# VitalyVorobyev/calibration

Measured on AMD Instinct MI355X. Metric: residual+Jacobian evals/sec, higher is better.
Workload: dtype f64

## Files before the change

calibration_amd/csrc/backend_hip.hip:

```cpp
#include <rccl/rccl.h>

#include <atomic>
#include <cstring>
#include <mutex>
#include <thread>
#include <set>

#include "engine.hpp"
#include "pipelines.hpp"
#include "lm_core.hpp"
#include "lm_state.hpp"
#include "lm_kernels.hpp"

namespace cba {


static inline unsigned nblk(int64_t n, int per) { return static_cast<unsigned>(std::max<int64_t>(1, (n + per - 1) / per)); }

template <class F>
struct ScopeExit {
    F f;
    ~ScopeExit() { f(); }
};
template <class F>
// ... 739 lines not shown
    st->pin_pack[1].reserve(e.pk_size);
    {
        hipFuncAttributes fa;
        (void)hipFuncGetAttributes(&fa, reinterpret_cast<const void*>(k_schur_view));
        warm_reproj_kernels();
    }
    if (const char* env = std::getenv("CBA_SYRK_MFMA")) st->syrk_mfma = std::atoi(env);
    if (const char* env = cba_exp_env("CBA_SCHUR_WAVE")) st->schur_wave = std::atoi(env);
    if (const char* env = cba_exp_env("CBA_LM_FUSE")) st->fuse_small = std::atoi(env);
    if (const char* env = cba_exp_env("CBA_LM_CTL_EVENT")) st->ctl_event = std::atoi(env);
    if (const char* env = cba_exp_env("CBA_SYNC_SPIN")) st->sync_spin = std::atoi(env);
    if (const char* env = std::getenv("CBA_LM_GRAPH")) {
        const int v = std::atoi(env);
        st->graphs_ok = v != 0;
        st->graph_after = v > 1 ? v : (v == 1 ? 0 : st->graph_after);
    }
    e.blk_w.alloc(std::max(1, s.n_blocks));
    e.cam_acc.alloc(static_cast<size_t>(s.n_cams) * s.NACC);
    e.view_L.alloc(nv * 36);
    e.view_y.alloc(nv * 6);
    e.view_D.alloc(nv * 6);
    e.view_gp.alloc(nv * 6);
    e.view_scale2.alloc(nv * 6);
    e.view_fixed.alloc(nv);
    e.view_fixed.zero(e.stream);
    e.blk_Z.alloc(static_cast<size_t>(std::max(1, s.n_blocks)) * 6 * s.PSH);
    e.blk_Z.zero(e.stream);
    up64(st->cam_off, s.cam_off);
    st->res_active.alloc(std::max(1, s.nsh));
    st->res_cam_var.alloc(std::max(1, s.n_cams));
    st->res_Hcc.alloc(static_cast<size_t>(s.nsh) * s.nsh);
    st->res_Ssch.alloc(static_cast<size_t>(s.nsh) * s.nsh);
    st->res_out.alloc(32);
    if (const char* env = cba_exp_env("CBA_LM_CTL")) st->lm_ctl_mode = std::atoi(env) != 0;
    if (const char* env = cba_exp_env("CBA_LM_CTL_POLL_US")) st->ctl_poll_us = std::atoi(env);
    if (const char* env = cba_exp_env("CBA_LM_PRELAUNCH")) st->ctl_prelaunch = std::atoi(env);
    if (const char* env = std::getenv("CBA_RCCL_TIMEOUT_S")) st->rccl_timeout_s = std::max(1, std::atoi(env));
    warm_lm_ctl();
    if (const char* env = std::getenv("CBA_LM_RESIDENT")) st->resident_mode = std::atoi(env);
    if (const char* env = std::getenv("CBA_LM_RESIDENT_MAX_OBS")) st->resident_max_obs = std::atoll(env);
    CBA_HIP(hipStreamSynchronize(e.stream));
}

void solve_stats(const Engine& e, int64_t stats8[8]) {
    const HipLMState* st = reinterpret_cast<const HipLMState*>(e.lm_state);
    for (int k = 0; k < 8; ++k) stats8[k] = st ? st->xs[k] : 0;
}

void set_lm_mode(Engine& e, int mode) {
    if (mode < 0 || mode > 3)
        throw std::invalid_argument("lm mode: 0 chip-wide kernels, 1 automatic, 2 resident kernel whenever possible, 3 chip-wide kernels with the host-side iteration (diagnosis)");
    lm_state(e)->resident_mode = mode == 3 ? 0 : mode;
    lm_state(e)->lm_ctl_mode = mode == 3 ? 0 : 1;
}


static LMDriver make_driver(Engine& e, HipBackend& be) {
    AllReduce ar = [&e](double* buf, int64_t n) { engine_allreduce(e, buf, n); };
    return LMDriver(lm_state(e)->s, be, e.h_intr, e.h_cam, e.h_view, e.h_target, ar, e.n_ranks, e.rank);
}

void warm_lm(Engine& e) {
    cba_options o{};
    o.max_iterations = 1;
    const bool resident = resident_lm_eligible(e, o);
    {
// ... 99 lines not shown
```

calibration_amd/csrc/lm_state.hpp:

```cpp
#pragma once
#include "engine.hpp"
#include "lm_ctl.hpp"
#include "schur_math.hpp"
#include "structure.hpp"

namespace cba {

struct HipLMState {
    Structure s;
    SchurDims dims;
    int n_vchunks = 0, n_tiles = 0, n_pairs = 0, n_cchunks = 0;
    int fuse_small = 1;
    int schur_wave = 1;
    int syrk_mfma = 1;
    DevBuf<int32_t> view_cam_blk, cam_blk;
    DevBuf<int64_t> cchunk_off, cam_seg, link_off;
    DevBuf<int32_t> link_blk;
    DevBuf<double> cam_partial, view_gmax, view_delta, view_stats, syrk_partial;
    PinnedBuf<double> pin, pin_ne, pin_tr;
    DevBuf<double> pack_dev, sys_tiles, stat_dev;
    PinnedBuf<double> pin_packed;
    hipEvent_t step_done = nullptr;
    hipEvent_t ctl_done = nullptr;
    int ctl_event = 0;
    int sync_spin = 1;
    ~HipLMState() {
        if (step_done) (void)hipEventDestroy(step_done);
        if (ctl_done) (void)hipEventDestroy(ctl_done);
    }
    int64_t xs[8] = {0, 0, 0, 0, 0, 0, 0, 0};
    struct GraphSlot {
        hipGraphExec_t exec = nullptr;
        double huber = 0.0;
        int constrained = -1, scalar = -1;
        int uses = 0;
        ~GraphSlot() { if (exec) (void)hipGraphExecDestroy(exec); }
    };
    GraphSlot g_new, g_schur, g_trial;
    bool graphs_ok = true;
    int graph_after = 200;
    PinnedBuf<double> pin_lmp;
    PinnedBuf<double> pin_pack[2];
    bool current_is_on_device = false;
    int resident_mode = 1;
    int64_t resident_max_obs = -1;
    DevBuf<int64_t> cam_off;
    DevBuf<int8_t> res_active, res_cam_var;
    DevBuf<double> res_Hcc, res_Ssch, res_out;
    PinnedBuf<double> pin_res;
    PinnedBuf<int8_t> pin_mask;
    DevBuf<double> ctl_buf;
    DevBuf<int32_t> ctl_idx;
    DevBuf<int8_t> ctl_eff;
    PinnedBuf<double> ctl_rec;
    CtlView ctl_view{};
    int ctl_n = -1;
    int rccl_timeout_s = 120;
    int ctl_prelaunch = 1;
    int ctl_poll_us = 2000;
    int lm_ctl_mode = 1;
};


inline HipLMState* lm_state(Engine& e) { return reinterpret_cast<HipLMState*>(e.lm_state); }

bool resident_lm_eligible(const Engine& e, const cba_options& o);
void resident_lm_warm(Engine& e);
bool resident_lm_solve(Engine& e, const cba_options& o, cba_summary* out, bool keep_parameters = false);

void launch_lm_ctl(const CtlView& V, int mode, int flag, hipStream_t stream);
bool lm_ctl_fits_lds(int n);
void warm_lm_ctl();

}
```

calibration_amd/csrc/resident_lm.hip:

```cpp
#include <chrono>
#include <cstdio>
#include <cstdlib>
#include <cstring>

#include "engine.hpp"
#include "lm_core.hpp"
#include "lm_state.hpp"
#include "mode_b.hpp"
#include "schur_math.hpp"

namespace cba {

constexpr int RES_THREADS = 512, RES_WAVES = RES_THREADS / 64;
constexpr int RES_NSH_MAX = 80;
constexpr int RES_MAX_CAMS = 16;
constexpr int RES_PROF = 16;

struct ResidentArgs {
    int n_blocks, n_cams, n_views, nsh, n_tiles, sh_base;
    SchurDims dims;
    const Tile* tiles;
    const int64_t *blk_tile_off, *link_off, *cam_off;
    const int32_t *blk_cam, *blk_view, *link_blk, *view_cam_blk, *cam_blk, *view_fixed;
    const double *X, *Y, *u, *v, *aux;
    double *bc, *sd;
    double *intr[2], *cam[2], *view[2], *target[2];
    double *partial, *blk_acc, *blk_s, *blk_w, *cam_acc;
    double *view_L, *view_y, *view_D, *view_gp, *view_scale2, *blk_Z, *view_delta;
    double *Hcc, *Ssch;
    const int8_t *active, *cam_var;
    int intr_var, target_var, constrained, line_search;
    double huber, eps;
    int max_iterations;
    double* out;
};

enum ResidentMsg { MSG_GRADIENT = 0, MSG_MAX_ITER, MSG_MIN_RADIUS, MSG_INVALID_STEPS, MSG_PARAMETER, MSG_FUNCTION, MSG_LINE_SEARCH };
static const char* const kResidentMsg[] = {"Gradient tolerance reached.", "Maximum number of iterations reached.",
                                           "Minimum trust region radius reached.",
                                           "Number of consecutive invalid steps more than max.", "Parameter tolerance reached.",
                                           "Function tolerance reached."};

struct ResidentShared {
    double A[RES_NSH_MAX][RES_NSH_MAX + 1];
    double rhs[RES_NSH_MAX], delta[RES_NSH_MAX], gc[RES_NSH_MAX], gsch[RES_NSH_MAX], scale2[RES_NSH_MAX];
    int idx[RES_NSH_MAX];
    int8_t eff[RES_NSH_MAX];
    double red[RES_WAVES][6];
    double grp[RES_THREADS];
    double radius, decrease_factor, cost, gmax, gmax_priv;
    int m, nfail, valid;
    unsigned long long prof[RES_PROF];
    double p_intr[2][RES_MAX_CAMS * 12], p_cam[2][RES_MAX_CAMS * 7], p_target[2][7];
};

template <int N>
__device__ __forceinline__ void block_sum(double (&v)[N], ResidentShared& sh) {
    const int lane = threadIdx.x & 63, wave = threadIdx.x >> 6;
#pragma unroll
    for (int k = 0; k < N; ++k) {
        const double t = wave_sum63(v[k]);
        if (lane == 63) sh.red[wave][k] = t;
    }
    __syncthreads();
#pragma unroll
    for (int k = 0; k < N; ++k) {
        double t = 0.0;
        for (int w = 0; w < RES_WAVES; ++w) t += sh.red[w][k];
        v[k] = t;
    }
    __syncthreads();
}

__device__ __forceinline__ double block_max(double v, ResidentShared& sh) {
    for (int o = 32; o > 0; o >>= 1) v = fmax(v, __shfl_xor(v, o));
    if ((threadIdx.x & 63) == 0) sh.red[threadIdx.x >> 6][0] = v;
    __syncthreads();
    double m = sh.red[0][0];
    for (int w = 1; w < RES_WAVES; ++w) m = fmax(m, sh.red[w][0]);
    __syncthreads();
    return m;
}

template <class NT, class TF, class OF>
// ... 122 lines not shown
        if (CHAIN == CH_INTRINSIC) {
            pA = a.view[which] + 7 * static_cast<int64_t>(a.blk_view[b]);
        } else if (CHAIN == CH_EXTRINSIC) {
            pA = a.view[which] + 7 * static_cast<int64_t>(a.blk_view[b]);
            pB = sh.p_cam[which] + 7 * a.blk_cam[b];
        } else {
            pA = sh.p_target[which];
            pB = sh.p_cam[which] + 7 * a.blk_cam[b];
            ax = a.aux + 12 * static_cast<int64_t>(b);
        }
        double o[BC_SIZE];
        block_consts<CHAIN>(pA, pB, ax, o);
        for (int i = 0; i < BC_SIZE; ++i) a.bc[static_cast<int64_t>(b) * BC_SIZE + i] = o[i];
    }
    if (MODEL == CAM_SCHEIMPFLUG)
        for (int c = threadIdx.x; c < a.n_cams; c += RES_THREADS) {
            double o[SD_SIZE];
            for (int i = 0; i < SD_SIZE; ++i) o[i] = 0.0;
            scheimpflug_consts(sh.p_intr[which] + 12 * c, o);
            for (int i = 0; i < SD_SIZE; ++i) a.sd[static_cast<int64_t>(c) * SD_SIZE + i] = o[i];
        }
    __syncthreads();
}

template <int CHAIN, int MODEL, int NPARTS, int PART>
struct ModeBParts {
    static __device__ __forceinline__ void run(const Tile t, int lane, const double* bcp, const double* ip, const double* sp,
                                               const ResidentArgs& a, double* row) {
        normal_eq_tile<CHAIN, MODEL, NPARTS, PART, double>(t, lane, bcp, ip, sp, a.X, a.Y, a.u, a.v, row);
        if constexpr (PART + 1 < NPARTS) ModeBParts<CHAIN, MODEL, NPARTS, PART + 1>::run(t, lane, bcp, ip, sp, a, row);
    }
};

template <int CHAIN, int MODEL>
__device__ __forceinline__ void phase_mode_b(const ResidentArgs& a) {
    constexpr int PI = IntrSize<MODEL>::value;
    constexpr int NACC = LocalCols<CHAIN, MODEL>::value * (LocalCols<CHAIN, MODEL>::value + 1) / 2 + LocalCols<CHAIN, MODEL>::value + 1;
    constexpr int NPARTS = CHAIN == CH_INTRINSIC ? 3 : 6;
    const int lane = threadIdx.x & 63;
    const int wave = __builtin_amdgcn_readfirstlane(threadIdx.x >> 6);
    const bool direct = a.n_tiles == a.n_blocks;
    for (int w = wave; w < a.n_tiles; w += RES_WAVES) {
        const Tile t = a.tiles[w];
        const int cam = a.blk_cam[t.blk];
        double* row = (direct ? a.blk_acc : a.partial) + static_cast<int64_t>(w) * NACC;
        ModeBParts<CHAIN, MODEL, NPARTS, 0>::run(t, lane, a.bc + static_cast<int64_t>(t.blk) * BC_SIZE, a.intr[0] + static_cast<int64_t>(cam) * PI,
                                                 a.sd + static_cast<int64_t>(cam) * SD_SIZE, a, row);
    }
    __syncthreads();
    if (!direct) {
        for (int idx = threadIdx.x; idx < a.n_blocks * NACC; idx += RES_THREADS) {
            const int b = idx / NACC, e = idx - b * NACC;
            double s = 0.0;
            for (int64_t t = a.blk_tile_off[b]; t < a.blk_tile_off[b + 1]; ++t) s += a.partial[t * NACC + e];
            a.blk_acc[idx] = s;
        }
        __syncthreads();
    }
}

template <int MODEL>
__device__ __forceinline__ double phase_resid_cost(const ResidentArgs& a, int which, ResidentShared& sh) {
    constexpr int PI = IntrSize<MODEL>::value;
    const int lane = threadIdx.x & 63;
    const int wave = __builtin_amdgcn_readfirstlane(threadIdx.x >> 6);
    for (int w = wave; w < a.n_tiles; w += RES_WAVES) {
        const Tile t = a.tiles[w];
        const int cam = a.blk_cam[t.blk];
        const double s = resid_tile<MODEL, double>(t, lane, a.bc + static_cast<int64_t>(t.blk) * BC_SIZE,
                                                   a.intr[which] + static_cast<int64_t>(cam) * PI, a.sd + static_cast<int64_t>(cam) * SD_SIZE,
                                                   a.X, a.Y, a.u, a.v);
        if (lane == 63) a.partial[w] = s;
    }
    __syncthreads();
    double c[1] = {0.0};
    for (int b = threadIdx.x; b < a.n_blocks; b += RES_THREADS) {
        double s = 0.0;
        for (int64_t t = a.blk_tile_off[b]; t < a.blk_tile_off[b + 1]; ++t) s += a.partial[t];
        a.blk_s[b] = s;
        double rho, w;
        huber(s, a.huber, &rho, &w);
        c[0] += 0.5 * rho;
    }
    block_sum(c, sh);
    return c[0];
}

__device__ __forceinline__ double phase_weights(const ResidentArgs& a, ResidentShared& sh) {
    const int NACC = a.dims.NACC, s_idx = a.dims.NH + a.dims.PL;
    double c[1] = {0.0};
    for (int b = threadIdx.x; b < a.n_blocks; b += RES_THREADS) {
        double rho, w;
        huber(a.blk_acc[static_cast<int64_t>(b) * NACC + s_idx], a.huber, &rho, &w);
        a.blk_w[b] = w;
        c[0] += 0.5 * rho;
    }
    block_sum(c, sh);
    grouped_sums(
        a.n_cams * NACC, [&](int idx) { const int cam = idx / NACC; return static_cast<int>(a.cam_off[cam + 1] - a.cam_off[cam]); },
        [&](int idx, int k) {
            const int cam = idx / NACC, e = idx - cam * NACC;
            const int b = a.cam_blk[a.cam_off[cam] + k];
            return a.blk_w[b] * a.blk_acc[static_cast<int64_t>(b) * NACC + e];
        },
        [&](int idx, double s) { a.cam_acc[idx] = s; }, sh);
    return c[0];
}

__device__ __forceinline__ void phase_assemble(const ResidentArgs& a, bool init_scale, ResidentShared& sh) {
    const int n = a.nsh, PL = a.dims.PL, NACC = a.dims.NACC, NH = a.dims.NH;
    for (int idx = threadIdx.x; idx < n * n + n; idx += RES_THREADS) {
        if (idx < n * n) {
            const int i = idx / n, j = idx - i * n;
            int ci, li, cj, lj;
            shared_decode(a, i, &ci, &li);
            shared_decode(a, j, &cj, &lj);
            double h = 0.0;
            if (ci < 0 && cj < 0) {
                for (int c = 0; c < a.n_cams; ++c) h += a.cam_acc[static_cast<int64_t>(c) * NACC + hidx_sym(PL, li, lj)];
            } else if (ci < 0 || cj < 0 || ci == cj) {
                h = a.cam_acc[static_cast<int64_t>(ci < 0 ? cj : ci) * NACC + hidx_sym(PL, li, lj)];
            }
            a.Hcc[idx] = h;
        } else {
            const int i = idx - n * n;
            int ci, li;
            shared_decode(a, i, &ci, &li);
            double g = 0.0;
            if (ci < 0) {
                for (int c = 0; c < a.n_cams; ++c) g += a.cam_acc[static_cast<int64_t>(c) * NACC + NH + li];
            } else {
                g = a.cam_acc[static_cast<int64_t>(ci) * NACC + NH + li];
            }
            sh.gc[i] = g;
        }
    }
    __syncthreads();
    for (int i = threadIdx.x; i < n; i += RES_THREADS) {
        const double hii = a.Hcc[static_cast<int64_t>(i) * n + i];
        sh.eff[i] = a.active[i] && hii != 0.0;
        if (init_scale) {
            const double sc = 1.0 / (1.0 + sqrt(hii));
            sh.scale2[i] = sc * sc;
        }
    }
    __syncthreads();
    if (threadIdx.x == 0) {
        int m = 0;
        for (int i = 0; i < n; ++i)
            if (sh.eff[i]) sh.idx[m++] = i;
        sh.m = m;
    }
}

template <class Tick>
__device__ __forceinline__ void phase_schur(const ResidentArgs& a, bool init_scale, ResidentShared& sh, Tick tick) {
    const int n = a.nsh;
    double gm = 0.0, nf[1] = {0.0};
    const double radius = sh.radius;
    for (int v = threadIdx.x; v < a.n_views; v += RES_THREADS) {
        const int nb = static_cast<int>(a.link_off[v + 1] - a.link_off[v]);
        double g = 0.0;
        const bool ok = schur_view_body(a.dims, nb, a.link_blk + a.link_off[v], a.blk_acc, a.blk_w, a.view_fixed[v] != 0, radius, init_scale,
                                        a.constrained != 0, a.view[0] + 7 * static_cast<int64_t>(v), a.view_scale2 + 6 * static_cast<int64_t>(v),
                                        a.view_L + 36 * static_cast<int64_t>(v), a.view_y + 6 * static_cast<int64_t>(v),
                                        a.view_D + 6 * static_cast<int64_t>(v), a.view_gp + 6 * static_cast<int64_t>(v), a.blk_Z, &g);
        if (ok) gm = fmax(gm, g);
        else nf[0] += 1.0;
    }
    tick(11);
    gm = block_max(gm, sh);
    block_sum(nf, sh);
    tick(12);
    if (threadIdx.x == 0) { sh.gmax_priv = gm; sh.nfail = static_cast<int>(nf[0] + 0.5); }
    const int PC = a.dims.PC, PSH = a.dims.PSH, n_cams = a.n_cams;
    grouped_sums(
        n * n, [&](int) { return a.n_views; },
        [&](int idx, int v) {
            const int i = idx / n, j = idx - i * n;
            const int ci = i / PC, cj = j / PC;
            const int bi = a.view_cam_blk[static_cast<int64_t>(v) * n_cams + ci], bj = a.view_cam_blk[static_cast<int64_t>(v) * n_cams + cj];
            if (bi < 0 || bj < 0) return 0.0;
            const double* zi = a.blk_Z + static_cast<int64_t>(bi) * 6 * PSH + (i - ci * PC);
            const double* zj = a.blk_Z + static_cast<int64_t>(bj) * 6 * PSH + (j - cj * PC);
            double s = 0.0;
#pragma unroll
            for (int k = 0; k < 6; ++k) s += zi[k * PSH] * zj[k * PSH];
            return s;
        },
        [&](int idx, double s) { a.Ssch[idx] = s; }, sh);
    tick(13);
    grouped_sums(
        n, [&](int) { return a.n_views; },
        [&](int i, int v) {
            const int ci = i / PC;
            const int bi = a.view_cam_blk[static_cast<int64_t>(v) * n_cams + ci];
// ... 84 lines not shown
}

template <int CHAIN, int MODEL>
__global__ __launch_bounds__(RES_THREADS) void k_resident_lm(const ResidentArgs a) {
    __shared__ ResidentShared sh;
    const int tid = threadIdx.x;
    const int n = a.nsh;
    const double eps = a.eps;
    constexpr double min_radius = 1e-32, max_radius = 1e16, min_rel_decrease = 1e-3;

    unsigned long long last = wall_clock64();
    auto tick = [&](int slot) {
        if (tid == 0) {
            const unsigned long long t = wall_clock64();
            sh.prof[slot] += t - last;
            last = t;
        }
    };
    {
        const int PI = IntrSize<MODEL>::value;
        for (int i = tid; i < a.n_cams * PI; i += RES_THREADS) {
            double x = a.intr[0][i];
            if (a.intr_var && i % PI < 2) x = fmax(x, 0.0);
            sh.p_intr[0][i] = x;
        }
        if (CHAIN != CH_INTRINSIC)
            for (int i = tid; i < a.n_cams * 7; i += RES_THREADS) sh.p_cam[0][i] = a.cam[0][i];
        if (CHAIN == CH_BUNDLE)
            for (int i = tid; i < 7; i += RES_THREADS) sh.p_target[0][i] = a.target[0][i];
        if (tid == 0) {
            for (int k = 0; k < RES_PROF; ++k) sh.prof[k] = 0;
            sh.radius = 1e4;
            sh.decrease_factor = 2.0;
        }
        __syncthreads();
        publish_shared(a, sh, 0, 0);
    }
    double initial_cost = 0.0;
    int iter = 0, invalid = 0, successful = 0, term = CBA_TERM_FAILURE, msg = MSG_INVALID_STEPS;
    bool linearise = true, re_eliminate = false, first = true;
    while (true) {
        if (linearise) {
            phase_consts<CHAIN, MODEL>(a, sh, 0);
            tick(0);
            phase_mode_b<CHAIN, MODEL>(a);
            tick(1);
            const double cost = phase_weights(a, sh);
            tick(2);
            phase_assemble(a, first, sh);
            tick(3);
            if (tid == 0) sh.cost = cost;
        }
        if (linearise || re_eliminate) {
            phase_schur(a, first && linearise, sh, tick);
            tick(4);
        }
        if (linearise) {
            const double gm_shared = shared_gmax(a, sh);
            if (tid == 0) sh.gmax = fmax(sh.gmax_priv, gm_shared);
            __syncthreads();
            tick(5);
        }
        linearise = re_eliminate = false;
        if (first) {
            first = false;
            initial_cost = sh.cost;
            if (sh.gmax <= eps) { term = CBA_TERM_CONVERGENCE; msg = MSG_GRADIENT; break; }
        }
        if (iter >= a.max_iterations) { term = CBA_TERM_NO_CONVERGENCE; msg = MSG_MAX_ITER; break; }
        if (sh.gmax <= eps) { term = CBA_TERM_CONVERGENCE; msg = MSG_GRADIENT; break; }
        if (sh.radius <= min_radius) { term = CBA_TERM_CONVERGENCE; msg = MSG_MIN_RADIUS; break; }
        ++iter;
        tick(10);
        phase_solve_reduced(a, sh);
        tick(6);
        bool valid = sh.valid != 0;
        if (valid) {
            double st[6] = {0.0, 0.0, 0.0, 0.0, 0.0, 0.0};
            shared_plus(a, sh, sh.delta, &st[0], &st[1]);
            for (int v = tid; v < a.n_views; v += RES_THREADS) {
                const int nb = static_cast<int>(a.link_off[v + 1] - a.link_off[v]);
                double o4[4];
                backsub_view_body(a.dims, nb, a.link_blk + a.link_off[v], a.blk_cam, a.blk_Z, sh.delta, a.view_fixed[v] != 0,
                                  a.view_L + 36 * static_cast<int64_t>(v), a.view_y + 6 * static_cast<int64_t>(v),
                                  a.view_D + 6 * static_cast<int64_t>(v), a.view_gp + 6 * static_cast<int64_t>(v),
                                  a.view[0] + 7 * static_cast<int64_t>(v), a.view_delta + 6 * static_cast<int64_t>(v),
                                  a.view[1] + 7 * static_cast<int64_t>(v), o4);
                for (int k = 0; k < 4; ++k) st[k] += o4[k];
            }
            for (int i = RES_THREADS - 1 - tid; i < n; i += RES_THREADS) {
                const double di = sh.delta[i];
                if (di != 0.0) {
                    st[4] += sh.gc[i] * di;
                    double s = 0.0;
                    for (int j = 0; j < n; ++j) s += a.Hcc[static_cast<int64_t>(i) * n + j] * sh.delta[j];
                    st[5] += di * s;
                }
            }
            block_sum(st, sh);
            tick(7);
            const double model_change = -(st[2] + st[4]) - 0.5 * (st[3] + st[5]);
            if (!(model_change > 0.0) || !(fabs(model_change) <= 1.7976931348623157e308)) valid = false;
            if (valid) {
                publish_shared(a, sh, 1, 1, false);
                phase_consts<CHAIN, MODEL>(a, sh, 1);
                double cand = phase_resid_cost<MODEL>(a, 1, sh);
                tick(8);
                if (!(fabs(cand) <= 1.7976931348623157e308)) cand = 1.7976931348623157e308;
                if (a.constrained && a.line_search && !(cand <= sh.cost + 1e-4 * (st[2] + st[4]))) { term = CBA_TERM_FAILURE; msg = MSG_LINE_SEARCH; break; }
                const double step_norm = sqrt(st[0]), x_norm = sqrt(st[1]);
                if (step_norm <= eps * (x_norm + eps)) { term = CBA_TERM_CONVERGENCE; msg = MSG_PARAMETER; break; }
                const double cost_change = sh.cost - cand;
                if (fabs(cost_change) <= eps * sh.cost) { term = CBA_TERM_CONVERGENCE; msg = MSG_FUNCTION; break; }
                const double rel = cost_change / model_change;
                invalid = 0;
                if (rel > min_rel_decrease) {
                    publish_shared(a, sh, 1, 0);
                    for (int i = tid; i < a.n_views * 7; i += RES_THREADS) a.view[0][i] = a.view[1][i];
                    ++successful;
                    __syncthreads();
                    if (tid == 0) {
                        const double t = 2.0 * rel - 1.0;
                        sh.radius = fmin(max_radius, sh.radius / fmax(1.0 / 3.0, 1.0 - t * t * t));
                        sh.decrease_factor = 2.0;
                    }
                    __syncthreads();
                    tick(9);
                    linearise = true;
                } else {
                    __syncthreads();
                    if (tid == 0) {
                        sh.radius = sh.radius / sh.decrease_factor;
                        sh.decrease_factor *= 2.0;
                    }
                    __syncthreads();
                    re_eliminate = true;
                }
                continue;
            }
        }
        if (++invalid >= 5) { term = CBA_TERM_FAILURE; msg = MSG_INVALID_STEPS; break; }
        __syncthreads();
        if (tid == 0) sh.radius *= 0.5;
        __syncthreads();
        re_eliminate = true;
    }
    __syncthreads();
    phase_consts<CHAIN, MODEL>(a, sh, 0);
    if (tid == 0) {
        a.out[0] = term;
        a.out[1] = iter;
        a.out[2] = successful;
        a.out[3] = initial_cost;
        a.out[4] = sh.cost;
        a.out[5] = msg;
        tick(10);
        for (int k = 0; k < RES_PROF; ++k) a.out[8 + k] = static_cast<double>(sh.prof[k]);
    }
}

bool resident_lm_eligible(const Engine& e, const cba_options& o) {
    const HipLMState* st = reinterpret_cast<const HipLMState*>(e.lm_state);
    if (!st || st->resident_mode == 0) return false;
    const Structure& s = st->s;
    if (e.n_ranks != 1 || e.allreduce || e.rccl_comm) return false;
    if (e.scalar != 0 || o.verbose) return false;
    if (s.n_blocks == 0 || s.nsh > RES_NSH_MAX || s.n_cams > RES_MAX_CAMS) return false;
    if (st->resident_mode == 1) {
        if (st->resident_max_obs >= 0) return s.n_obs <= st->resident_max_obs;
        if (s.chain == CBA_CHAIN_INTRINSIC) return 1.0 * s.n_views + 0.0105 * static_cast<double>(s.n_obs) <= 28.0;
        return false;
    }
    return true;
}

static ResidentArgs resident_args(Engine& e, HipLMState& st) {
    const Structure& s = st.s;
    ResidentArgs a{};
    a.n_blocks = s.n_blocks; a.n_cams = s.n_cams; a.n_views = s.n_views; a.nsh = s.nsh;
    a.n_tiles = static_cast<int>(e.n_tilesB); a.sh_base = s.sh_base;
    a.dims = st.dims;
    a.tiles = e.tilesB.p; a.blk_tile_off = e.d_blk_tile_off.p; a.link_off = st.link_off.p; a.cam_off = st.cam_off.p;
    a.blk_cam = e.d_blk_cam.p; a.blk_view = e.d_blk_view.p; a.link_blk = st.link_blk.p; a.view_cam_blk = st.view_cam_blk.p;
    a.cam_blk = st.cam_blk.p; a.view_fixed = e.view_fixed.p;
    a.X = e.X.p; a.Y = e.Y.p; a.u = e.u.p; a.v = e.v.p; a.aux = e.aux.p;
    a.bc = e.bc.p; a.sd = e.sd.p;
    for (int k = 0; k < 2; ++k) { a.intr[k] = e.intr[k].p; a.cam[k] = e.cam[k].p; a.view[k] = e.view[k].p; a.target[k] = e.target[k].p; }
    a.partial = e.partial.p; a.blk_acc = e.blk_acc.p; a.blk_s = e.blk_s.p; a.blk_w = e.blk_w.p; a.cam_acc = e.cam_acc.p;
    a.view_L = e.view_L.p; a.view_y = e.view_y.p; a.view_D = e.view_D.p; a.view_gp = e.view_gp.p; a.view_scale2 = e.view_scale2.p;
    a.blk_Z = e.blk_Z.p; a.view_delta = st.view_delta.p;
    a.Hcc = st.res_Hcc.p; a.Ssch = st.res_Ssch.p;
    a.active = st.res_active.p; a.cam_var = st.res_cam_var.p;
    a.out = st.res_out.p;
    return a;
}

static void resident_launch(Engine& e, const ResidentArgs& a) {
#define CALL(C, M) hipLaunchKernelGGL((k_resident_lm<C, M>), dim3(1), dim3(RES_THREADS), 0, e.stream, a);
    switch (e.chain * 2 + e.model) {
        case 0: CALL(CH_INTRINSIC, CAM_PINHOLE_BC) break;
        case 1: CALL(CH_INTRINSIC, CAM_SCHEIMPFLUG) break;
        case 2: CALL(CH_EXTRINSIC, CAM_PINHOLE_BC) break;
        case 3: CALL(CH_EXTRINSIC, CAM_SCHEIMPFLUG) break;
        case 4: CALL(CH_BUNDLE, CAM_PINHOLE_BC) break;
        case 5: CALL(CH_BUNDLE, CAM_SCHEIMPFLUG) break;
        default: throw std::runtime_error("bad chain/model");
    }
#undef CALL
    CBA_HIP(hipGetLastError());
}

void resident_lm_warm(Engine& e) {
    HipLMState& st = *lm_state(e);
    cba_options o{};
    o.max_iterations = 0;
    o.huber_delta = 1.0;
    o.epsilon = 1e-9;
    if (!resident_lm_eligible(e, o)) return;
    cba_summary s{};
    resident_lm_solve(e, o, &s, true);
    (void)st;
// ... 33 lines not shown
    a.huber = o.huber_delta; a.eps = o.epsilon; a.max_iterations = o.max_iterations;
    a.line_search = 1;
    if (const char* env = std::getenv("CBA_LM_LINE_SEARCH")) a.line_search = std::atoi(env) != 0;
    resident_launch(e, a);
    const size_t n_intr = e.h_intr.size(), n_cam = e.h_cam.size(), n_view = e.h_view.size();
    st.pin_res.reserve(8 + n_intr + n_cam + 7 + n_view + RES_PROF);
    double* p = st.pin_res.p;
    st.res_out.download(p, 8, e.stream);
    double* prof = p + 8 + n_intr + n_cam + 7 + n_view;
    st.res_out.download(prof, RES_PROF, e.stream, 8);
    e.intr[0].download(p + 8, n_intr, e.stream);
    if (e.chain != CBA_CHAIN_INTRINSIC) e.cam[0].download(p + 8 + n_intr, n_cam, e.stream);
    if (e.chain == CBA_CHAIN_BUNDLE) e.target[0].download(p + 8 + n_intr + n_cam, 7, e.stream);
    if (n_view) e.view[0].download(p + 8 + n_intr + n_cam + 7, n_view, e.stream);
    CBA_HIP(hipStreamSynchronize(e.stream));
    e.active = 0;
    if (static_cast<int>(p[5]) == MSG_LINE_SEARCH) {
        if (!e.h_view.empty()) e.view[0].upload(e.h_view.data(), e.h_view.size(), e.stream);
        e.intr[0].upload(e.h_intr.data(), e.h_intr.size(), e.stream);
        if (e.chain != CBA_CHAIN_INTRINSIC) e.cam[0].upload(e.h_cam.data(), e.h_cam.size(), e.stream);
        if (e.chain == CBA_CHAIN_BUNDLE) e.target[0].upload(e.h_target.data(), 7, e.stream);
        CBA_HIP(hipStreamSynchronize(e.stream));
        return false;
    }
    if (!keep_parameters) {
        std::memcpy(e.h_intr.data(), p + 8, sizeof(double) * n_intr);
        if (e.chain != CBA_CHAIN_INTRINSIC) std::memcpy(e.h_cam.data(), p + 8 + n_intr, sizeof(double) * n_cam);
        if (e.chain == CBA_CHAIN_BUNDLE) std::memcpy(e.h_target.data(), p + 8 + n_intr + n_cam, sizeof(double) * 7);
        if (n_view) std::memcpy(e.h_view.data(), p + 8 + n_intr + n_cam + 7, sizeof(double) * n_view);
    }
    if (std::getenv("CBA_LM_RESIDENT_PROFILE")) {
        static const char* const names[RES_PROF] = {"consts", "mode B", "weights + camera sums", "assemble", "schur", "gradient norm",
                                                    "reduced solve", "trial step", "trial cost", "accept", "control", "schur: views",
                                                    "schur: max", "schur: S", "", ""};
        std::fprintf(stderr, "[cba] resident LM phases (us):");
        for (int k = 0; k < RES_PROF - 2; ++k) std::fprintf(stderr, " %s %.1f |", names[k], prof[k] * 0.01);
        std::fprintf(stderr, "\n");
    }
    const int term = static_cast<int>(p[0]), msg = static_cast<int>(p[5]);
    out->termination = term;
    out->success = term == CBA_TERM_CONVERGENCE;
    out->iterations = static_cast<int>(p[1]);
    out->successful_steps = static_cast<int>(p[2]);
    out->initial_cost = p[3];
    out->final_cost = p[4];
    out->solve_seconds = std::chrono::duration<double>(std::chrono::steady_clock::now() - t0).count();
    std::snprintf(out->report, sizeof(out->report), "calibba(schur LM, resident kernel): %s iters=%d cost %.6e -> %.6e",
                  kResidentMsg[msg >= 0 && msg < 6 ? msg : 3], out->iterations, out->initial_cost, out->final_cost);
    return true;
}

}
```

Baseline: 27.72 billion.

## Speculatively linearise at trial point in resident LM with double-buffered block accumulators

Each trial step in the resident LM kernel now runs the full mode-B Jacobian accumulation at the trial parameters instead of only computing the residual cost. The block accumulators and weights are double-buffered, so an accepted step flips a selector and reuses the trial linearisation instead of recomputing it. For the intrinsic chain, mode-B work is split into fixed 128-point units processed by wave pairs that exchange Jacobian rows through LDS, with next-unit loads prefetched. The trade is extra work on rejected steps (speculation is turned off after a rejection) plus additional device buffers and a larger shared-memory union.

New measurement: 27.71 billion, median of 4. About the same (-0.0%).

```diff
diff --git a/calibration_amd/csrc/backend_hip.hip b/calibration_amd/csrc/backend_hip.hip
--- a/calibration_amd/csrc/backend_hip.hip
+++ b/calibration_amd/csrc/backend_hip.hip
@@ -795,6 +795,7 @@
     st->res_Hcc.alloc(static_cast<size_t>(s.nsh) * s.nsh);
     st->res_Ssch.alloc(static_cast<size_t>(s.nsh) * s.nsh);
     st->res_out.alloc(32);
+    resident_lm_init(e);
     if (const char* env = cba_exp_env("CBA_LM_CTL")) st->lm_ctl_mode = std::atoi(env) != 0;
     if (const char* env = cba_exp_env("CBA_LM_CTL_POLL_US")) st->ctl_poll_us = std::atoi(env);
     if (const char* env = cba_exp_env("CBA_LM_PRELAUNCH")) st->ctl_prelaunch = std::atoi(env);
diff --git a/calibration_amd/csrc/lm_state.hpp b/calibration_amd/csrc/lm_state.hpp
--- a/calibration_amd/csrc/lm_state.hpp
+++ b/calibration_amd/csrc/lm_state.hpp
@@ -47,6 +47,10 @@
     DevBuf<int64_t> cam_off;
     DevBuf<int8_t> res_active, res_cam_var;
     DevBuf<double> res_Hcc, res_Ssch, res_out;
+    DevBuf<Tile> res_units;
+    DevBuf<int32_t> res_blk_unit_off;
+    DevBuf<double> res_rows;
+    int res_n_units = 0;
     PinnedBuf<double> pin_res;
     PinnedBuf<int8_t> pin_mask;
     DevBuf<double> ctl_buf;
@@ -64,6 +68,7 @@
 
 inline HipLMState* lm_state(Engine& e) { return reinterpret_cast<HipLMState*>(e.lm_state); }
 
+void resident_lm_init(Engine& e);
 bool resident_lm_eligible(const Engine& e, const cba_options& o);
 void resident_lm_warm(Engine& e);
 bool resident_lm_solve(Engine& e, const cba_options& o, cba_summary* out, bool keep_parameters = false);
diff --git a/calibration_amd/csrc/resident_lm.hip b/calibration_amd/csrc/resident_lm.hip
--- a/calibration_amd/csrc/resident_lm.hip
+++ b/calibration_amd/csrc/resident_lm.hip
@@ -14,6 +14,9 @@
 constexpr int RES_THREADS = 512, RES_WAVES = RES_THREADS / 64;
 constexpr int RES_NSH_MAX = 80;
 constexpr int RES_MAX_CAMS = 16;
+constexpr int RES_PAIRS = RES_WAVES / 2;
+constexpr int RES_UNIT = 128;
+constexpr int RES_ROW_NR2 = 16;
 constexpr int RES_PROF = 16;
 
 struct ResidentArgs {
@@ -25,7 +28,11 @@
     const double *X, *Y, *u, *v, *aux;
     double *bc, *sd;
     double *intr[2], *cam[2], *view[2], *target[2];
-    double *partial, *blk_acc, *blk_s, *blk_w, *cam_acc;
+    double *blk_acc[2], *blk_w[2], *sub[2];
+    double *partial, *blk_s, *cam_acc;
+    const Tile* units;
+    const int32_t* blk_unit_off;
+    int n_units;
     double *view_L, *view_y, *view_D, *view_gp, *view_scale2, *blk_Z, *view_delta;
     double *Hcc, *Ssch;
     const int8_t *active, *cam_var;
@@ -41,8 +48,13 @@
                                            "Number of consecutive invalid steps more than max.", "Parameter tolerance reached.",
                                            "Function tolerance reached."};
 
+typedef double res_v2 __attribute__((ext_vector_type(2)));
+
 struct ResidentShared {
-    double A[RES_NSH_MAX][RES_NSH_MAX + 1];
+    union {
+        double A[RES_NSH_MAX][RES_NSH_MAX + 1];
+        res_v2 rows[RES_WAVES][RES_ROW_NR2][64];
+    };
     double rhs[RES_NSH_MAX], delta[RES_NSH_MAX], gc[RES_NSH_MAX], gsch[RES_NSH_MAX], scale2[RES_NSH_MAX];
     int idx[RES_NSH_MAX];
     int8_t eff[RES_NSH_MAX];
@@ -50,6 +62,7 @@
     double grp[RES_THREADS];
     double radius, decrease_factor, cost, gmax, gmax_priv;
     int m, nfail, valid;
+    int sel;
     unsigned long long prof[RES_PROF];
     double p_intr[2][RES_MAX_CAMS * 12], p_cam[2][RES_MAX_CAMS * 7], p_target[2][7];
 };
@@ -238,30 +251,120 @@
     }
 };
 
+__device__ __forceinline__ void lds_barrier() {
+    __builtin_amdgcn_fence(__ATOMIC_RELEASE, "workgroup", "local");
+    __builtin_amdgcn_s_barrier();
+    __builtin_amdgcn_fence(__ATOMIC_ACQUIRE, "workgroup", "local");
+}
+
+template <int MODEL, int PART>
+__device__ __forceinline__ void mode_b_pair_wave(const ResidentArgs& a, ResidentShared& sh, int which, double* rows_out, int pair, int lane) {
+    using D = DirectRows<CH_INTRINSIC, MODEL>;
+    using SPLIT = SplitRoundRobin<2>;
+    constexpr int PI = D::PI, PL = D::PL, NACC = PL * (PL + 1) / 2 + PL + 1, NR2 = (D::N + 1) / 2;
+    constexpr int NLOC = SPLIT::count(PL, PART), NPAD = TransposeSum<16>::pad(NLOC);
+    static_assert(NR2 <= RES_ROW_NR2, "row buffers of ResidentShared");
+    res_v2(*mine)[64] = sh.rows[2 * pair + PART];
+    const res_v2(*theirs)[64] = sh.rows[2 * pair + (PART ^ 1)];
+    const int rounds = (a.n_units + RES_PAIRS - 1) / RES_PAIRS;
+    const int j = PART * 64 + lane, jo = (PART ^ 1) * 64 + lane;
+    const auto* blk_cam = (const __attribute__((address_space(4))) int32_t*)a.blk_cam;
+    auto units = [&](int i) {
+        const auto* p = (const __attribute__((address_space(4))) int64_t*)(a.units + i);
+        const int64_t w0 = p[0];
+        return Tile{static_cast<int32_t>(w0 & 0xffffffff), static_cast<int32_t>(w0 >> 32), p[1], p[2], 0};
+    };
+    const Tile none{0, 0, 0, 0, 0};
+    Tile t = pair < a.n_units ? units(pair) : none;
+    int cam = blk_cam[t.blk];
+    double x = 0.0, y = 0.0, u = 0.0, v = 0.0;
+    if (j < t.count) { x = a.X[t.xy_start + j]; y = a.Y[t.xy_start + j]; u = a.u[t.start + j]; v = a.v[t.start + j]; }
+#pragma unroll 1
+    for (int r = 0; r < rounds; ++r) {
+        const int ui = r * RES_PAIRS + pair;
+        const Tile tn = ui + RES_PAIRS < a.n_units ? units(ui + RES_PAIRS) : none;
+        const int camn = blk_cam[tn.blk];
+        double xn = 0.0, yn = 0.0, un = 0.0, vn = 0.0;
+        if (j < tn.count) { xn = a.X[tn.xy_start + j]; yn = a.Y[tn.xy_start + j]; un = a.u[tn.start + j]; vn = a.v[tn.start + j]; }
+        double acc[NPAD];
+#pragma unroll
+        for (int e = 0; e < NPAD; ++e) acc[e] = 0.0;
+        if (j < t.count) {
+            double w[2 * NR2];
+            direct_rows<CH_INTRINSIC, MODEL, double>(a.bc + static_cast<int64_t>(t.blk) * BC_SIZE, a.intr[which] + static_cast<int64_t>(cam) * PI,
+                                                     a.sd + static_cast<int64_t>(cam) * SD_SIZE, x, y, u, v, w);
+            if (D::N & 1) w[D::N] = 0.0;
+#pragma unroll
+            for (int k = 0; k < NR2; ++k) mine[k][lane] = res_v2{w[2 * k], w[2 * k + 1]};
+            direct_accumulate<CH_INTRINSIC, MODEL, SPLIT, PART>(w, acc);
+        }
+        lds_barrier();
+        if (jo < t.count) {
+            double w[2 * NR2];
+#pragma unroll
+            for (int k = 0; k < NR2; ++k) { const res_v2 d = theirs[k][lane]; w[2 * k] = d.x; w[2 * k + 1] = d.y; }
+            direct_accumulate<CH_INTRINSIC, MODEL, SPLIT, PART>(w, acc);
+        }
+        if (t.count > 0) {
+            bool owner;
+            const int base = wave_transpose_sum<NPAD>(acc, lane, &owner);
+            double* out = rows_out + static_cast<int64_t>(ui) * NACC;
+#pragma unroll
+            for (int jj = 0; jj < TransposeSum<NPAD>::CNT; ++jj) {
+                const int l = base + jj;
+                if (owner && l < NLOC) {
+                    const int e = SPLIT::entry(PL, PART, l);
+                    if (e < NACC) out[e] = acc[jj];
+                }
+            }
+        }
+        lds_barrier();
+        t = tn; cam = camn; x = xn; y = yn; u = un; v = vn;
+    }
+}
+
 template <int CHAIN, int MODEL>
-__device__ __forceinline__ void phase_mode_b(const ResidentArgs& a) {
+__device__ __forceinline__ void phase_mode_b(const ResidentArgs& a, ResidentShared& sh, int which, int set) {
     constexpr int PI = IntrSize<MODEL>::value;
     constexpr int NACC = LocalCols<CHAIN, MODEL>::value * (LocalCols<CHAIN, MODEL>::value + 1) / 2 + LocalCols<CHAIN, MODEL>::value + 1;
-    constexpr int NPARTS = CHAIN == CH_INTRINSIC ? 3 : 6;
     const int lane = threadIdx.x & 63;
     const int wave = __builtin_amdgcn_readfirstlane(threadIdx.x >> 6);
-    const bool direct = a.n_tiles == a.n_blocks;
-    for (int w = wave; w < a.n_tiles; w += RES_WAVES) {
-        const Tile t = a.tiles[w];
-        const int cam = a.blk_cam[t.blk];
-        double* row = (direct ? a.blk_acc : a.partial) + static_cast<int64_t>(w) * NACC;
-        ModeBParts<CHAIN, MODEL, NPARTS, 0>::run(t, lane, a.bc + static_cast<int64_t>(t.blk) * BC_SIZE, a.intr[0] + static_cast<int64_t>(cam) * PI,
-                                                 a.sd + static_cast<int64_t>(cam) * SD_SIZE, a, row);
-    }
-    __syncthreads();
-    if (!direct) {
-        for (int idx = threadIdx.x; idx < a.n_blocks * NACC; idx += RES_THREADS) {
-            const int b = idx / NACC, e = idx - b * NACC;
-            double s = 0.0;
-            for (int64_t t = a.blk_tile_off[b]; t < a.blk_tile_off[b + 1]; ++t) s += a.partial[t * NACC + e];
-            a.blk_acc[idx] = s;
-        }
+    double* const acc = a.blk_acc[set];
+    double* const sub = a.sub[set];
+    if constexpr (CHAIN == CH_INTRINSIC) {
+        const bool direct = a.n_units == a.n_blocks;
+        if (wave & 1) mode_b_pair_wave<MODEL, 1>(a, sh, which, direct ? acc : sub, wave >> 1, lane);
+        else mode_b_pair_wave<MODEL, 0>(a, sh, which, direct ? acc : sub, wave >> 1, lane);
         __syncthreads();
+        if (!direct) {
+            for (int idx = threadIdx.x; idx < a.n_blocks * NACC; idx += RES_THREADS) {
+                const int b = idx / NACC, e = idx - b * NACC;
+                double s = 0.0;
+                for (int u = a.blk_unit_off[b]; u < a.blk_unit_off[b + 1]; ++u) s += sub[static_cast<int64_t>(u) * NACC + e];
+                acc[idx] = s;
+            }
+            __syncthreads();
+        }
+    } else {
+        constexpr int NPARTS = 6;
+        const bool direct = a.n_tiles == a.n_blocks;
+        for (int w = wave; w < a.n_tiles; w += RES_WAVES) {
+            const Tile t = a.tiles[w];
+            const int cam = a.blk_cam[t.blk];
+            double* row = (direct ? acc : sub) + static_cast<int64_t>(w) * NACC;
+            ModeBParts<CHAIN, MODEL, NPARTS, 0>::run(t, lane, a.bc + static_cast<int64_t>(t.blk) * BC_SIZE, a.intr[which] + static_cast<int64_t>(cam) * PI,
+                                                     a.sd + static_cast<int64_t>(cam) * SD_SIZE, a, row);
+        }
+        __syncthreads();
+        if (!direct) {
+            for (int idx = threadIdx.x; idx < a.n_blocks * NACC; idx += RES_THREADS) {
+                const int b = idx / NACC, e = idx - b * NACC;
+                double s = 0.0;
+                for (int64_t t = a.blk_tile_off[b]; t < a.blk_tile_off[b + 1]; ++t) s += sub[t * NACC + e];
+                acc[idx] = s;
+            }
+            __syncthreads();
+        }
     }
 }
 
@@ -292,25 +395,33 @@
     return c[0];
 }
 
-__device__ __forceinline__ double phase_weights(const ResidentArgs& a, ResidentShared& sh) {
+__device__ __forceinline__ double phase_weights(const ResidentArgs& a, int set, ResidentShared& sh) {
     const int NACC = a.dims.NACC, s_idx = a.dims.NH + a.dims.PL;
+    const double* blk_acc = a.blk_acc[set];
+    double* blk_w = a.blk_w[set];
     double c[1] = {0.0};
     for (int b = threadIdx.x; b < a.n_blocks; b += RES_THREADS) {
         double rho, w;
-        huber(a.blk_acc[static_cast<int64_t>(b) * NACC + s_idx], a.huber, &rho, &w);
-        a.blk_w[b] = w;
+        huber(blk_acc[static_cast<int64_t>(b) * NACC + s_idx], a.huber, &rho, &w);
+        blk_w[b] = w;
         c[0] += 0.5 * rho;
     }
     block_sum(c, sh);
+    return c[0];
+}
+
+__device__ __forceinline__ void phase_camera_sums(const ResidentArgs& a, int set, ResidentShared& sh) {
+    const int NACC = a.dims.NACC;
+    const double* blk_acc = a.blk_acc[set];
+    const double* blk_w = a.blk_w[set];
     grouped_sums(
         a.n_cams * NACC, [&](int idx) { const int cam = idx / NACC; return static_cast<int>(a.cam_off[cam + 1] - a.cam_off[cam]); },
         [&](int idx, int k) {
             const int cam = idx / NACC, e = idx - cam * NACC;
             const int b = a.cam_blk[a.cam_off[cam] + k];
-            return a.blk_w[b] * a.blk_acc[static_cast<int64_t>(b) * NACC + e];
+            return blk_w[b] * blk_acc[static_cast<int64_t>(b) * NACC + e];
         },
         [&](int idx, double s) { a.cam_acc[idx] = s; }, sh);
-    return c[0];
 }
 
 __device__ __forceinline__ void phase_assemble(const ResidentArgs& a, bool init_scale, ResidentShared& sh) {
@@ -360,14 +471,14 @@
 }
 
 template <class Tick>
-__device__ __forceinline__ void phase_schur(const ResidentArgs& a, bool init_scale, ResidentShared& sh, Tick tick) {
+__device__ __forceinline__ void phase_schur(const ResidentArgs& a, int set, bool init_scale, ResidentShared& sh, Tick tick) {
     const int n = a.nsh;
     double gm = 0.0, nf[1] = {0.0};
     const double radius = sh.radius;
     for (int v = threadIdx.x; v < a.n_views; v += RES_THREADS) {
         const int nb = static_cast<int>(a.link_off[v + 1] - a.link_off[v]);
         double g = 0.0;
-        const bool ok = schur_view_body(a.dims, nb, a.link_blk + a.link_off[v], a.blk_acc, a.blk_w, a.view_fixed[v] != 0, radius, init_scale,
+        const bool ok = schur_view_body(a.dims, nb, a.link_blk + a.link_off[v], a.blk_acc[set], a.blk_w[set], a.view_fixed[v] != 0, radius, init_scale,
                                         a.constrained != 0, a.view[0] + 7 * static_cast<int64_t>(v), a.view_scale2 + 6 * static_cast<int64_t>(v),
                                         a.view_L + 36 * static_cast<int64_t>(v), a.view_y + 6 * static_cast<int64_t>(v),
                                         a.view_D + 6 * static_cast<int64_t>(v), a.view_gp + 6 * static_cast<int64_t>(v), a.blk_Z, &g);
@@ -518,80 +629,37 @@
             for (int k = 0; k < RES_PROF; ++k) sh.prof[k] = 0;
             sh.radius = 1e4;
             sh.decrease_factor = 2.0;
+            sh.sel = 0;
         }
         __syncthreads();
         publish_shared(a, sh, 0, 0);
     }
     double initial_cost = 0.0;
     int iter = 0, invalid = 0, successful = 0, term = CBA_TERM_FAILURE, msg = MSG_INVALID_STEPS;
-    bool linearise = true, re_eliminate = false, first = true;
+    bool evaluate = true, trial = false, speculate = true, re_eliminate = false, first = true;
+    double st[6] = {0.0, 0.0, 0.0, 0.0, 0.0, 0.0}, model_change = 0.0;
     while (true) {
-        if (linearise) {
-            phase_consts<CHAIN, MODEL>(a, sh, 0);
-            tick(0);
-            phase_mode_b<CHAIN, MODEL>(a);
-            tick(1);
-            const double cost = phase_weights(a, sh);
-            tick(2);
-            phase_assemble(a, first, sh);
-            tick(3);
-            if (tid == 0) sh.cost = cost;
-        }
-        if (linearise || re_eliminate) {
-            phase_schur(a, first && linearise, sh, tick);
-            tick(4);
-        }
-        if (linearise) {
-            const double gm_shared = shared_gmax(a, sh);
-            if (tid == 0) sh.gmax = fmax(sh.gmax_priv, gm_shared);
-            __syncthreads();
-            tick(5);
-        }
-        linearise = re_eliminate = false;
-        if (first) {
-            first = false;
-            initial_cost = sh.cost;
-            if (sh.gmax <= eps) { term = CBA_TERM_CONVERGENCE; msg = MSG_GRADIENT; break; }
-        }
-        if (iter >= a.max_iterations) { term = CBA_TERM_NO_CONVERGENCE; msg = MSG_MAX_ITER; break; }
-        if (sh.gmax <= eps) { term = CBA_TERM_CONVERGENCE; msg = MSG_GRADIENT; break; }
-        if (sh.radius <= min_radius) { term = CBA_TERM_CONVERGENCE; msg = MSG_MIN_RADIUS; break; }
-        ++iter;
-        tick(10);
-        phase_solve_reduced(a, sh);
-        tick(6);
-        bool valid = sh.valid != 0;
-        if (valid) {
-            double st[6] = {0.0, 0.0, 0.0, 0.0, 0.0, 0.0};
-            shared_plus(a, sh, sh.delta, &st[0], &st[1]);
-            for (int v = tid; v < a.n_views; v += RES_THREADS) {
-                const int nb = static_cast<int>(a.link_off[v + 1] - a.link_off[v]);
-                double o4[4];
-                backsub_view_body(a.dims, nb, a.link_blk + a.link_off[v], a.blk_cam, a.blk_Z, sh.delta, a.view_fixed[v] != 0,
-                                  a.view_L + 36 * static_cast<int64_t>(v), a.view_y + 6 * static_cast<int64_t>(v),
-                                  a.view_D + 6 * static_cast<int64_t>(v), a.view_gp + 6 * static_cast<int64_t>(v),
-                                  a.view[0] + 7 * static_cast<int64_t>(v), a.view_delta + 6 * static_cast<int64_t>(v),
-                                  a.view[1] + 7 * static_cast<int64_t>(v), o4);
-                for (int k = 0; k < 4; ++k) st[k] += o4[k];
-            }
-            for (int i = RES_THREADS - 1 - tid; i < n; i += RES_THREADS) {
-                const double di = sh.delta[i];
-                if (di != 0.0) {
-                    st[4] += sh.gc[i] * di;
-                    double s = 0.0;
-                    for (int j = 0; j < n; ++j) s += a.Hcc[static_cast<int64_t>(i) * n + j] * sh.delta[j];
-                    st[5] += di * s;
-                }
-            }
-            block_sum(st, sh);
-            tick(7);
-            const double model_change = -(st[2] + st[4]) - 0.5 * (st[3] + st[5]);
-            if (!(model_change > 0.0) || !(fabs(model_change) <= 1.7976931348623157e308)) valid = false;
-            if (valid) {
-                publish_shared(a, sh, 1, 1, false);
-                phase_consts<CHAIN, MODEL>(a, sh, 1);
-                double cand = phase_resid_cost<MODEL>(a, 1, sh);
+        bool new_system = false;
+        if (evaluate) {
+            const int which = trial ? 1 : 0;
+            const bool full = !trial || speculate;
+            const int set = trial ? sh.sel ^ 1 : sh.sel;
+            double cand;
+            phase_consts<CHAIN, MODEL>(a, sh, which);
+            if (!trial) tick(0);
+            if (full) {
+                phase_mode_b<CHAIN, MODEL>(a, sh, which, set);
+                if (!trial) tick(1);
+                cand = phase_weights(a, set, sh);
+                tick(trial ? 14 : 2);
+            } else {
+                cand = phase_resid_cost<MODEL>(a, 1, sh);
                 tick(8);
+            }
+            if (!trial) {
+                if (tid == 0) sh.cost = cand;
+                new_system = true;
+            } else {
                 if (!(fabs(cand) <= 1.7976931348623157e308)) cand = 1.7976931348623157e308;
                 if (a.constrained && a.line_search && !(cand <= sh.cost + 1e-4 * (st[2] + st[4]))) { term = CBA_TERM_FAILURE; msg = MSG_LINE_SEARCH; break; }
                 const double step_norm = sqrt(st[0]), x_norm = sqrt(st[1]);
@@ -609,10 +677,14 @@
                         const double t = 2.0 * rel - 1.0;
                         sh.radius = fmin(max_radius, sh.radius / fmax(1.0 / 3.0, 1.0 - t * t * t));
                         sh.decrease_factor = 2.0;
+                        if (full) { sh.sel ^= 1; sh.cost = cand; }
                     }
                     __syncthreads();
                     tick(9);
-                    linearise = true;
+                    trial = false;
+                    speculate = true;
+                    if (!full) continue;
+                    new_system = true;
                 } else {
                     __syncthreads();
                     if (tid == 0) {
@@ -621,7 +693,70 @@
                     }
                     __syncthreads();
                     re_eliminate = true;
+                    speculate = false;
                 }
+            }
+        }
+        evaluate = trial = false;
+        if (new_system) {
+            phase_camera_sums(a, sh.sel, sh);
+            tick(2);
+            phase_assemble(a, first, sh);
+            tick(3);
+        }
+        if (new_system || re_eliminate) {
+            phase_schur(a, sh.sel, first && new_system, sh, tick);
+            tick(4);
+        }
+        if (new_system) {
+            const double gm_shared = shared_gmax(a, sh);
+            if (tid == 0) sh.gmax = fmax(sh.gmax_priv, gm_shared);
+            __syncthreads();
+            tick(5);
+        }
+        re_eliminate = false;
+        if (first) {
+            first = false;
+            initial_cost = sh.cost;
+            if (sh.gmax <= eps) { term = CBA_TERM_CONVERGENCE; msg = MSG_GRADIENT; break; }
+        }
+        if (iter >= a.max_iterations) { term = CBA_TERM_NO_CONVERGENCE; msg = MSG_MAX_ITER; break; }
+        if (sh.gmax <= eps) { term = CBA_TERM_CONVERGENCE; msg = MSG_GRADIENT; break; }
+        if (sh.radius <= min_radius) { term = CBA_TERM_CONVERGENCE; msg = MSG_MIN_RADIUS; break; }
+        ++iter;
+        tick(10);
+        phase_solve_reduced(a, sh);
+        tick(6);
+        bool valid = sh.valid != 0;
+        if (valid) {
+            for (int k = 0; k < 6; ++k) st[k] = 0.0;
+            shared_plus(a, sh, sh.delta, &st[0], &st[1]);
+            for (int v = tid; v < a.n_views; v += RES_THREADS) {
+                const int nb = static_cast<int>(a.link_off[v + 1] - a.link_off[v]);
+                double o4[4];
+                backsub_view_body(a.dims, nb, a.link_blk + a.link_off[v], a.blk_cam, a.blk_Z, sh.delta, a.view_fixed[v] != 0,
+                                  a.view_L + 36 * static_cast<int64_t>(v), a.view_y + 6 * static_cast<int64_t>(v),
+                                  a.view_D + 6 * static_cast<int64_t>(v), a.view_gp + 6 * static_cast<int64_t>(v),
+                                  a.view[0] + 7 * static_cast<int64_t>(v), a.view_delta + 6 * static_cast<int64_t>(v),
+                                  a.view[1] + 7 * static_cast<int64_t>(v), o4);
+                for (int k = 0; k < 4; ++k) st[k] += o4[k];
+            }
+            for (int i = RES_THREADS - 1 - tid; i < n; i += RES_THREADS) {
+                const double di = sh.delta[i];
+                if (di != 0.0) {
+                    st[4] += sh.gc[i] * di;
+                    double s = 0.0;
+                    for (int j = 0; j < n; ++j) s += a.Hcc[static_cast<int64_t>(i) * n + j] * sh.delta[j];
+                    st[5] += di * s;
+                }
+            }
+            block_sum(st, sh);
+            tick(7);
+            model_change = -(st[2] + st[4]) - 0.5 * (st[3] + st[5]);
+            if (!(model_change > 0.0) || !(fabs(model_change) <= 1.7976931348623157e308)) valid = false;
+            if (valid) {
+                publish_shared(a, sh, 1, 1, false);
+                evaluate = trial = true;
                 continue;
             }
         }
@@ -630,6 +765,7 @@
         if (tid == 0) sh.radius *= 0.5;
         __syncthreads();
         re_eliminate = true;
+        speculate = false;
     }
     __syncthreads();
     phase_consts<CHAIN, MODEL>(a, sh, 0);
@@ -658,6 +794,32 @@
         return false;
     }
     return true;
+}
+
+void resident_lm_init(Engine& e) {
+    HipLMState& st = *lm_state(e);
+    const Structure& s = st.s;
+    if (s.n_blocks == 0) return;
+    if (e.blk_acc_alt.n < e.blk_acc.n) { e.blk_acc_alt.alloc(e.blk_acc.n); e.blk_w_alt.alloc(e.blk_w.n); }
+    const size_t NACC = static_cast<size_t>(st.dims.NACC);
+    if (e.chain != CBA_CHAIN_INTRINSIC) {
+        st.res_rows.alloc(static_cast<size_t>(e.n_tilesB) * NACC);
+        return;
+    }
+    std::vector<Tile> units;
+    std::vector<int32_t> off(static_cast<size_t>(s.n_blocks) + 1, 0);
+    for (int b = 0; b < s.n_blocks; ++b) {
+        const int64_t nb = e.blk_offset[b + 1] - e.blk_offset[b];
+        for (int64_t k = 0; k < nb; k += RES_UNIT)
+            units.push_back(Tile{b, static_cast<int32_t>(std::min<int64_t>(RES_UNIT, nb - k)), e.pad_offset[b] + k, e.xy_offset[b] + k, 0});
+        off[b + 1] = static_cast<int32_t>(units.size());
+    }
+    st.res_n_units = static_cast<int>(units.size());
+    if (units.empty()) units.push_back(Tile{0, 0, 0, 0, 0});
+    st.res_units.assign(units.data(), units.size(), e.stream);
+    st.res_blk_unit_off.assign(off.data(), off.size(), e.stream);
+    st.res_rows.alloc(2 * units.size() * NACC);
+    CBA_HIP(hipStreamSynchronize(e.stream));
 }
 
 static ResidentArgs resident_args(Engine& e, HipLMState& st) {
@@ -672,7 +834,15 @@
     a.X = e.X.p; a.Y = e.Y.p; a.u = e.u.p; a.v = e.v.p; a.aux = e.aux.p;
     a.bc = e.bc.p; a.sd = e.sd.p;
     for (int k = 0; k < 2; ++k) { a.intr[k] = e.intr[k].p; a.cam[k] = e.cam[k].p; a.view[k] = e.view[k].p; a.target[k] = e.target[k].p; }
-    a.partial = e.partial.p; a.blk_acc = e.blk_acc.p; a.blk_s = e.blk_s.p; a.blk_w = e.blk_w.p; a.cam_acc = e.cam_acc.p;
+    a.partial = e.partial.p; a.blk_s = e.blk_s.p; a.cam_acc = e.cam_acc.p;
+    a.blk_acc[0] = e.blk_acc.p; a.blk_acc[1] = e.blk_acc_alt.p; a.blk_w[0] = e.blk_w.p; a.blk_w[1] = e.blk_w_alt.p;
+    if (e.chain == CBA_CHAIN_INTRINSIC) {
+        a.units = st.res_units.p; a.blk_unit_off = st.res_blk_unit_off.p; a.n_units = st.res_n_units;
+        a.sub[0] = st.res_rows.p;
+        a.sub[1] = st.res_rows.p + static_cast<size_t>(st.res_n_units) * static_cast<size_t>(st.dims.NACC);
+    } else {
+        a.sub[0] = e.partial.p; a.sub[1] = st.res_rows.p;
+    }
     a.view_L = e.view_L.p; a.view_y = e.view_y.p; a.view_D = e.view_D.p; a.view_gp = e.view_gp.p; a.view_scale2 = e.view_scale2.p;
     a.blk_Z = e.blk_Z.p; a.view_delta = st.view_delta.p;
     a.Hcc = st.res_Hcc.p; a.Ssch = st.res_Ssch.p;
@@ -772,9 +942,9 @@
     if (std::getenv("CBA_LM_RESIDENT_PROFILE")) {
         static const char* const names[RES_PROF] = {"consts", "mode B", "weights + camera sums", "assemble", "schur", "gradient norm",
                                                     "reduced solve", "trial step", "trial cost", "accept", "control", "schur: views",
-                                                    "schur: max", "schur: S", "", ""};
+                                                    "schur: max", "schur: S", "trial linearisation", ""};
         std::fprintf(stderr, "[cba] resident LM phases (us):");
-        for (int k = 0; k < RES_PROF - 2; ++k) std::fprintf(stderr, " %s %.1f |", names[k], prof[k] * 0.01);
+        for (int k = 0; k < RES_PROF - 1; ++k) std::fprintf(stderr, " %s %.1f |", names[k], prof[k] * 0.01);
         std::fprintf(stderr, "\n");
     }
     const int term = static_cast<int>(p[0]), msg = static_cast<int>(p[5]);
```
